# jaco267/polar-code-pytorch-sionna

Hardware: NVIDIA B200
Metric: decoded_info_throughput_sc_n1024 (higher is better)
Workload: dtype f32

## Files before the change

### polar-code-pytorch-sionna_b200/csrc/polar_sc5.cu

```cuda
#include <atomic>
#include <mutex>

#include "polar_common.cuh"
#include "polar_internal.h"

namespace polar {

#if !defined(POLAR_F_BOXPLUS)
namespace {
__global__ void nsmid_kernel(unsigned *out) {
  unsigned v;
  asm volatile("mov.u32 %0, %%nsmid;" : "=r"(v));
  *out = v;
}
std::mutex g_scr_mu;
std::atomic<float *> g_scr_buf[64];
}

int sc_scratch_init(int device) {
  if (device < 0 || device >= 64) return set_error(POLAR_EINVAL, "init: bad device %d", device);
  std::lock_guard<std::mutex> lk(g_scr_mu);
  if (g_scr_buf[device].load(std::memory_order_acquire)) return POLAR_OK;
  unsigned *d_n = nullptr, h_n = 0;
  POLAR_CUDA(cudaMalloc(&d_n, sizeof(unsigned)));
  nsmid_kernel<<<1, 1>>>(d_n);
  const cudaError_t e = cudaMemcpy(&h_n, d_n, sizeof(unsigned), cudaMemcpyDeviceToHost);
  cudaFree(d_n);
  if (e != cudaSuccess) return set_error(POLAR_ECUDA, "init: %s", cudaGetErrorString(e));
  if (h_n == 0 || h_n > 1024) return set_error(POLAR_ECUDA, "init: implausible %%nsmid = %u", h_n);
  void *p = nullptr;
  if (cudaMalloc(&p, (size_t)h_n * kScScratchPerSm) != cudaSuccess) {
    (void)cudaGetLastError();
    return set_error(POLAR_ENOMEM, "init: cudaMalloc of the %zu-byte SC stage scratch failed", (size_t)h_n * kScScratchPerSm);
  }
  g_scr_buf[device].store((float *)p, std::memory_order_release);
  return POLAR_OK;
}
float *sc_scratch() {
  int dev = 0;
  if (cudaGetDevice(&dev) != cudaSuccess || dev < 0 || dev >= 64) return nullptr;
  return g_scr_buf[dev].load(std::memory_order_acquire);
}
#endif

__device__ unsigned long long g_sc5_dbg[8];

namespace {

constexpr unsigned FULLMASK = 0xFFFFFFFFu;
constexpr int kSlotFloats = 1024, kSlotBytes = 4096;
constexpr int kSlots = 6;
constexpr int kHeaderBytes = 1024;

#define SC5_T(slot)                                                                   \
  do {                                                                                \
    if (DBG && threadIdx.x == 0 && blockIdx.x == 0) {                                 \
      const long long t__ = clock64(); g_sc5_dbg[slot] += (unsigned long long)(t__ - tlast); tlast = t__; \
    }                                                                                 \
  } while (0)

struct Ctl {
  unsigned long long bar[8 * kSlots];
  uint32_t tm_addr;
  uint32_t pad[3];
};
static_assert(sizeof(Ctl) + 128 + 8 <= kHeaderBytes, "sc5: header");

struct Sc5Layout {
  int nw, nws, n64, stride, slots;
  size_t fmask_off, nz_off, warp_off, per_warp, beta_off, total;
};
__host__ __device__ inline Sc5Layout sc5_layout(int m, int warps, int slots) {
  Sc5Layout l;
  const int n = 1 << m;
  l.nw = n >> 5; l.nws = l.nw + 1; l.n64 = n >> 7; l.slots = slots;
  l.stride = 128 + 4;
  l.fmask_off = (sizeof(Ctl) + 15) / 16 * 16;
  l.nz_off = l.fmask_off + (size_t)l.nw * 4;
  l.warp_off = (l.nz_off + (size_t)l.n64 + 1023) / 1024 * 1024;
  l.beta_off = (size_t)slots * kSlotBytes > (size_t)32 * l.stride * 4 ? (size_t)slots * kSlotBytes : (size_t)32 * l.stride * 4;
  l.per_warp = (l.beta_off + (size_t)32 * l.nws * 4 + 127) / 128 * 128;
  l.total = l.warp_off + (size_t)warps * l.per_warp;
  return l;
}

PDEV uint32_t smem_u32(const void *p) { return (uint32_t)__cvta_generic_to_shared(p); }
PDEV void mbar_init(unsigned long long *bar, uint32_t count) {
  asm volatile("mbarrier.init.shared::cta.b64 [%0], %1;" ::"r"(smem_u32(bar)), "r"(count) : "memory");
}
PDEV void mbar_expect_tx(unsigned long long *bar, uint32_t bytes) {
  asm volatile("mbarrier.arrive.expect_tx.shared::cta.b64 _, [%0], %1;" ::"r"(smem_u32(bar)), "r"(bytes) : "memory");
}
PDEV void mbar_wait(unsigned long long *bar, uint32_t parity) {
  asm volatile(
      "{\n\t"
      ".reg .pred P1;\n\t"
      "SC5_WAIT:\n\t"
      "mbarrier.try_wait.parity.shared::cta.b64 P1, [%0], %1, %2;\n\t"
      "@P1 bra SC5_DONE;\n\t"
      "bra SC5_WAIT;\n\t"
      "SC5_DONE:\n\t"
      "}" ::"r"(smem_u32(bar)), "r"(parity), "r"(0x989680u) : "memory");
}
PDEV void bulk_g2s(void *dst, const void *src, uint32_t bytes, unsigned long long *bar, uint64_t policy) {
  asm volatile("cp.async.bulk.shared::cluster.global.mbarrier::complete_tx::bytes.L2::cache_hint [%0], [%1], %2, [%3], %4;"
               ::"r"(smem_u32(dst)), "l"(src), "r"(bytes), "r"(smem_u32(bar)), "l"(policy) : "memory");
}
PDEV uint64_t l2_policy_evict_last() {
  uint64_t p; asm volatile("createpolicy.fractional.L2::evict_last.b64 %0, 1.0;" : "=l"(p)); return p;
}
PDEV uint64_t l2_policy_evict_first() {
  uint64_t p; asm volatile("createpolicy.fractional.L2::evict_first.b64 %0, 1.0;" : "=l"(p)); return p;
}
PDEV uint64_t l2_policy_evict_normal() {
  uint64_t p; asm volatile("createpolicy.fractional.L2::evict_normal.b64 %0, 1.0;" : "=l"(p)); return p;
}
PDEV void stg4_hint(float *p, const float4 v, uint64_t policy) {
  asm volatile("st.global.L2::cache_hint.v4.f32 [%0], {%1, %2, %3, %4}, %5;"
               ::"l"(p), "f"(v.x), "f"(v.y), "f"(v.z), "f"(v.w), "l"(policy) : "memory");
}
PDEV float4 lds4(const float *p) { return *reinterpret_cast<const float4 *>(p); }
PDEV void sts4(float *p, float4 v) { *reinterpret_cast<float4 *>(p) = v; }
PDEV float4 f4(const float4 a, const float4 b) {
  float4 o;
  o.x = f_minsum(a.x, b.x); o.y = f_minsum(a.y, b.y); o.z = f_minsum(a.z, b.z); o.w = f_minsum(a.w, b.w);
  return o;
}
PDEV float4 f4nc(const float4 a, const float4 b) {
  float4 o;
  o.x = f_minsum_noclip(a.x, b.x); o.y = f_minsum_noclip(a.y, b.y); o.z = f_minsum_noclip(a.z, b.z); o.w = f_minsum_noclip(a.w, b.w);
  return o;
}
PDEV float4 f4neg(const float4 a, const float4 b) {
  float4 o;
  o.x = f_minsum_neg(a.x, b.x); o.y = f_minsum_neg(a.y, b.y); o.z = f_minsum_neg(a.z, b.z); o.w = f_minsum_neg(a.w, b.w);
  return o;
}
PDEV float4 g4(const float4 a, const float4 b, const uint32_t bits) {
  float4 o;
  o.x = g_minsum(a.x, b.x, (bits << 31) & 0x80000000u);
  o.y = g_minsum(a.y, b.y, (bits << 30) & 0x80000000u);
  o.z = g_minsum(a.z, b.z, (bits << 29) & 0x80000000u);
  o.w = g_minsum(a.w, b.w, (bits << 28) & 0x80000000u);
  return o;
}
PDEV float gneg(float a, float b, uint32_t signmask) { return u2f(f2u(a) ^ signmask ^ 0x80000000u) - b; }
PDEV float4 g4neg(const float4 a, const float4 b, const uint32_t bits) {
  float4 o;
  o.x = gneg(a.x, b.x, (bits << 31) & 0x80000000u);
  o.y = gneg(a.y, b.y, (bits << 30) & 0x80000000u);
  o.z = gneg(a.z, b.z, (bits << 29) & 0x80000000u);
  o.w = gneg(a.w, b.w, (bits << 28) & 0x80000000u);
  return o;
}

PDEV void tmem_st8(uint32_t taddr, const float4 a, const float4 b) {
  asm volatile("tcgen05.st.sync.aligned.32x32b.x8.b32 [%0], {%1, %2, %3, %4, %5, %6, %7, %8};"
               ::"r"(taddr), "r"(f2u(a.x)), "r"(f2u(a.y)), "r"(f2u(a.z)), "r"(f2u(a.w)), "r"(f2u(b.x)), "r"(f2u(b.y)),
               "r"(f2u(b.z)), "r"(f2u(b.w)) : "memory");
}
PDEV void tmem_st4(uint32_t taddr, const float4 a) {
  asm volatile("tcgen05.st.sync.aligned.32x32b.x4.b32 [%0], {%1, %2, %3, %4};"
               ::"r"(taddr), "r"(f2u(a.x)), "r"(f2u(a.y)), "r"(f2u(a.z)), "r"(f2u(a.w)) : "memory");
}
PDEV void tmem_wait_st() { asm volatile("tcgen05.wait::st.sync.aligned;" ::: "memory"); }
struct Tm8 { uint32_t r[8]; };
PDEV void tmem_ld8_issue(uint32_t taddr, Tm8 &v) {
  asm volatile("tcgen05.ld.sync.aligned.32x32b.x8.b32 {%0, %1, %2, %3, %4, %5, %6, %7}, [%8];"
               : "=r"(v.r[0]), "=r"(v.r[1]), "=r"(v.r[2]), "=r"(v.r[3]), "=r"(v.r[4]), "=r"(v.r[5]), "=r"(v.r[6]), "=r"(v.r[7])
               : "r"(taddr) : "memory");
}
PDEV void tmem_ld_wait(Tm8 &a, Tm8 &b) {
  asm volatile("tcgen05.wait::ld.sync.aligned;"
               : "+r"(a.r[0]), "+r"(a.r[1]), "+r"(a.r[2]), "+r"(a.r[3]), "+r"(a.r[4]), "+r"(a.r[5]), "+r"(a.r[6]), "+r"(a.r[7]),
                 "+r"(b.r[0]), "+r"(b.r[1]), "+r"(b.r[2]), "+r"(b.r[3]), "+r"(b.r[4]), "+r"(b.r[5]), "+r"(b.r[6]), "+r"(b.r[7])
               :: "memory");
}
PDEV float4 tm_lo(const Tm8 &v) { return make_float4(u2f(v.r[0]), u2f(v.r[1]), u2f(v.r[2]), u2f(v.r[3])); }
PDEV float4 tm_hi(const Tm8 &v) { return make_float4(u2f(v.r[4]), u2f(v.r[5]), u2f(v.r[6]), u2f(v.r[7])); }

template <int D, bool FIRST_G, bool FROM_CH, int NS>
__device__ __noinline__ void descent(const float *__restrict__ src, const int nvalid, const uint32_t *beta, const int nws,
                                     const int left_word, float *scr, const uint32_t tm_base, float *Lw, const uint32_t bar_a,
                                     uint32_t &par, const int lane, const bool discard) {
  constexpr int NB = 1 << D;
  constexpr int HB = NB / 2;
  constexpr int SRC = 256 * NB;
  constexpr bool WIDE = D <= 2;
  constexpr int CPS = D == 1 ? 2 : 1;
  constexpr int NQ = WIDE ? 1 : (1 << (D - 3));
  constexpr int K = WIDE ? 32 / CPS : 64 * NQ;
  constexpr int T1 = 8 + D - 1;
  const uint64_t pol_src = FROM_CH ? l2_policy_evict_first() : (D == 1 ? l2_policy_evict_last() : l2_policy_evict_normal());
  const uint64_t pol_s9 = l2_policy_evict_last(), pol_sx = l2_policy_evict_normal();
  if (!FROM_CH) asm volatile("fence.proxy.async.global;" ::: "memory");
  asm volatile("fence.proxy.async.shared::cta;" ::: "memory");
  __syncwarp();
  const uint32_t slot_a = smem_u32(Lw);

  auto issue2 = [&](const int k, const int ring) {
    if (WIDE) {
      if (lane < 2) {
        const int s = ring + lane;
        int c = (k + lane) * CPS;
        if (FROM_CH && c >= nvalid) c = nvalid - 1;
        asm volatile("mbarrier.arrive.expect_tx.shared::cta.b64 _, [%0], %1;" ::"r"(bar_a + 8 * s), "r"(4096) : "memory");
        asm volatile("cp.async.bulk.shared::cluster.global.mbarrier::complete_tx::bytes.L2::cache_hint [%0], [%1], %2, [%3], %4;"
                     ::"r"(slot_a + 4096 * s), "l"(src + (size_t)c * SRC), "r"(4096), "r"(bar_a + 8 * s), "l"(pol_src) : "memory");
      }
    } else {
      if (lane < 2)
        asm volatile("mbarrier.arrive.expect_tx.shared::cta.b64 _, [%0], %1;" ::"r"(bar_a + 8 * (ring + lane)), "r"(4096) : "memory");
      __syncwarp();
      if (lane < 16) {
        const int h = lane >> 3, p = lane & 7, s = ring + h;
        int c = k / (2 * NQ);
        const int q = (k >> 1) % NQ;
        if (FROM_CH && c >= nvalid) c = nvalid - 1;
        const int blk = (p & 3) + 4 * q + ((p >> 2) ? HB : 0);
        asm volatile("cp.async.bulk.shared::cluster.global.mbarrier::complete_tx::bytes.L2::cache_hint [%0], [%1], %2, [%3], %4;"
                     ::"r"(slot_a + 4096 * s + 512 * p), "l"(src + (size_t)c * SRC + blk * 256 + h * 128), "r"(512), "r"(bar_a + 8 * s),
                     "l"(pol_src) : "memory");
      }
    }
  };
  auto wait = [&](const int s) -> const float * {
    asm volatile(
        "{\n\t"
        ".reg .pred P1;\n\t"
        "SC5_WAIT:\n\t"
        "mbarrier.try_wait.parity.shared::cta.b64 P1, [%0], %1, %2;\n\t"
        "@P1 bra SC5_DONE;\n\t"
        "bra SC5_WAIT;\n\t"
        "SC5_DONE:\n\t"
        "}" ::"r"(bar_a + 8 * s), "r"((par >> s) & 1u), "r"(0x989680u) : "memory");
    return Lw + s * kSlotFloats;
  };

#pragma unroll
  for (int r = 0; r < NS; r += 2) issue2(r, r);
  int ring = 0;
  const int col = 4 * lane;
  float *st1 = scr + (size_t)32 * ((1 << T1) - 512) + col;
  const uint32_t *bp = beta + left_word + (col >> 5);
  const int sh = col & 31;
  const float *dp = src + lane * 32;
  if constexpr (WIDE) {
    constexpr int CW = 2 * CPS;
    int tcol = 0;
#pragma unroll 1
    for (int k = 0; k < K; k += 2) {
      const float *sl[2];
      sl[0] = wait(ring); sl[1] = wait(ring + 1);
      float4 v[CW][2][NB];
#pragma unroll
      for (int u = 0; u < CW; ++u)
#pragma unroll
        for (int e = 0; e < 2; ++e)
#pragma unroll
          for (int i = 0; i < NB; ++i) v[u][e][i] = lds4(sl[u / CPS] + (u % CPS) * SRC + i * 256 + col + 128 * e);
      float4 out[CW][2];
#pragma unroll
      for (int u = 0; u < CW; ++u) {
#pragma unroll
        for (int e = 0; e < 2; ++e) {
          float4 r1[HB];
#pragma unroll
          for (int i = 0; i < HB; ++i) {
            if (FIRST_G) {
              const uint32_t bits = bp[u * nws + i * 8 + e * 4] >> sh;
              r1[i] = FROM_CH ? g4neg(v[u][e][i], v[u][e][i + HB], bits) : g4(v[u][e][i], v[u][e][i + HB], bits);
            } else {
              r1[i] = FROM_CH ? f4neg(v[u][e][i], v[u][e][i + HB]) : f4(v[u][e][i], v[u][e][i + HB]);
            }
            if (D >= 2) stg4_hint(st1 + u * (1 << T1) + i * 256 + e * 128, r1[i], T1 == 9 ? pol_s9 : pol_sx);
          }
          if (D == 2) out[u][e] = FIRST_G ? f4(r1[0], r1[HB - 1]) : f4nc(r1[0], r1[HB - 1]);
          else out[u][e] = r1[0];
        }
      }
      if (!FROM_CH && discard) {
        asm volatile("discard.global.L2 [%0], 128;" ::"l"(dp) : "memory");
        asm volatile("discard.global.L2 [%0], 128;" ::"l"(dp + 1024) : "memory");
      }
      st1 += CW << T1; bp += CW * nws; dp += 2048;
      __syncwarp();
      par ^= 3u << ring;
      if (k + NS < K) issue2(k + NS, ring);
#pragma unroll
      for (int u = 0; u < CW; ++u) tmem_st8(tm_base + tcol + 8 * u, out[u][0], out[u][1]);
      tcol += 8 * CW;
      ring = (ring + 2 == NS) ? 0 : ring + 2;
    }
  } else {
    const int piece = (lane >> 2) & 7, line = lane & 3;
    dp = src + ((piece & 3) + ((piece >> 2) ? HB : 0)) * 256 + line * 32;
#pragma unroll 1
    for (int c = 0; c < 32; ++c) {
      float4 R[2][HB];
#pragma unroll
      for (int q = 0; q < NQ; ++q) {
        const int k = (c * NQ + q) * 2;
        const float *sl[2];
        sl[0] = wait(ring); sl[1] = wait(ring + 1);
        float4 v[2][8];
#pragma unroll
        for (int h = 0; h < 2; ++h)
#pragma unroll
          for (int p = 0; p < 8; ++p) v[h][p] = lds4(sl[h] + p * 128 + col);
#pragma unroll
        for (int h = 0; h < 2; ++h) {
#pragma unroll
          for (int t = 0; t < 4; ++t) {
            const int blk = 4 * q + t;
            if (FIRST_G) {
              const uint32_t bits = bp[blk * 8 + h * 4] >> sh;
              R[h][blk] = FROM_CH ? g4neg(v[h][t], v[h][4 + t], bits) : g4(v[h][t], v[h][4 + t], bits);
            } else {
              R[h][blk] = FROM_CH ? f4neg(v[h][t], v[h][4 + t]) : f4(v[h][t], v[h][4 + t]);
            }
            stg4_hint(st1 + blk * 256 + h * 128, R[h][blk], T1 == 9 ? pol_s9 : pol_sx);
          }
        }
        if (!FROM_CH && discard) {
          asm volatile("discard.global.L2 [%0], 128;" ::"l"(dp + 4 * q * 256) : "memory");
          asm volatile("discard.global.L2 [%0], 128;" ::"l"(dp + 4 * q * 256 + 128) : "memory");
        }
        __syncwarp();
        par ^= 3u << ring;
        if (k + NS < K) issue2(k + NS, ring);
        ring = (ring + 2 == NS) ? 0 : ring + 2;
      }
#pragma unroll
      for (int lv = D - 1; lv >= 1; --lv) {
        const int half = 1 << (lv - 1);
        float *stl = scr + (size_t)32 * ((1 << (8 + lv - 1)) - 512) + (size_t)c * (1 << (8 + lv - 1)) + col;
#pragma unroll
        for (int h = 0; h < 2; ++h)
#pragma unroll
          for (int i = 0; i < half; ++i) {
            R[h][i] = (FIRST_G && lv == D - 1) ? f4(R[h][i], R[h][i + half]) : f4nc(R[h][i], R[h][i + half]);
            if (lv - 1 >= 1) stg4_hint(stl + i * 256 + h * 128, R[h][i], (8 + lv - 1) == 9 ? pol_s9 : pol_sx);
          }
      }
      tmem_st8(tm_base + 8 * c, R[0][0], R[1][0]);
      st1 += 1 << T1; bp += nws; dp += SRC;
    }
  }
  tmem_wait_st();
  __syncwarp();
}

template <bool IS_G>
PDEV void step_tmem(float *L, const uint32_t *beta, const int stride, const int nws, const int lane, const uint32_t tm_base,
                    const int left_word) {
  const int j = lane << 2;
  const uint32_t *bp = beta + left_word + (j >> 5);
  const int sh = j & 31;
  float *dst = L + j;
  Tm8 a0, a1, a2, a3, b0, b1, b2, b3;
  auto issue4 = [&](const int k0, Tm8 &v0, Tm8 &v1, Tm8 &v2, Tm8 &v3) {
    tmem_ld8_issue(tm_base + 8 * k0, v0);
    tmem_ld8_issue(tm_base + 8 * (k0 + 1), v1);
    tmem_ld8_issue(tm_base + 8 * (k0 + 2), v2);
    tmem_ld8_issue(tm_base + 8 * (k0 + 3), v3);
  };
  auto compute4 = [&](const int k0, const Tm8 &v0, const Tm8 &v1, const Tm8 &v2, const Tm8 &v3) {
#pragma unroll
    for (int r = 0; r < 4; ++r) {
      const Tm8 &v = r == 0 ? v0 : r == 1 ? v1 : r == 2 ? v2 : v3;
      const float4 a = tm_lo(v), b = tm_hi(v);
      float4 o;
      if (IS_G) o = g4(a, b, bp[(k0 + r) * nws] >> sh);
      else o = f4(a, b);
      sts4(dst + (k0 + r) * stride, o);
    }
  };
  issue4(0, a0, a1, a2, a3);
#pragma unroll 1
  for (int k0 = 0; k0 < 32; k0 += 8) {
    tmem_ld_wait(a0, a1); tmem_ld_wait(a2, a3);
    issue4(k0 + 4, b0, b1, b2, b3);
    compute4(k0, a0, a1, a2, a3);
    tmem_ld_wait(b0, b1); tmem_ld_wait(b2, b3);
    if (k0 + 8 < 32) issue4(k0 + 8, a0, a1, a2, a3);
    compute4(k0 + 4, b0, b1, b2, b3);
  }
}

PDEV uint64_t tree64(const float (&x)[64], uint64_t fm) {
  uint32_t bl = 0, bc = 0;
#pragma unroll 1
  for (int h = 0; h < 2; ++h) {
    const uint32_t fmc = h ? (uint32_t)(fm >> 32) : (uint32_t)fm;
    if (fmc == FULLMASK) { bc = 0; continue; }
    float y[32];
#pragma unroll
    for (int j = 0; j < 32; ++j)
      y[j] = h ? g_minsum(x[j], x[j + 32], (bl << (31 - j)) & 0x80000000u) : f_minsum(x[j], x[j + 32]);
    bc = BetaTree<5>::run(y, fmc);
    if (h == 0) bl = bc;
  }
  return (uint64_t)(bl ^ bc) | ((uint64_t)bc << 32);
}
PDEV uint4 bottom128(const float *node, uint64_t fm0, uint64_t fm1) {
  uint64_t bl = 0, bc = 0;
#pragma unroll 1
  for (int h = 0; h < 2; ++h) {
    const uint64_t fmc = h ? fm1 : fm0;
    if (fmc == ~0ull) { bc = 0; continue; }
    float x[64];
#pragma unroll
    for (int q = 0; q < 16; ++q) {
      const float4 a = lds4(node + 4 * q), b = lds4(node + 64 + 4 * q);
      const float4 o = h ? g4(a, b, (uint32_t)(bl >> (4 * q))) : f4(a, b);
      x[4 * q] = o.x; x[4 * q + 1] = o.y; x[4 * q + 2] = o.z; x[4 * q + 3] = o.w;
    }
    bc = tree64(x, fmc);
    if (h == 0) bl = bc;
  }
  const uint64_t lo = bl ^ bc;
  return make_uint4((uint32_t)lo, (uint32_t)(lo >> 32), (uint32_t)bc, (uint32_t)(bc >> 32));
}

template <int M, int NS, bool DBG>
__global__ void __launch_bounds__(256, 1) sc5_kernel(const float *__restrict__ logit, const uint32_t *__restrict__ fmask_g,
                                                     int64_t B, int64_t nbatches, float *scratch, size_t scratch_per_sm,
                                                     int scr_discard, uint32_t *__restrict__ u_packed, float *__restrict__ u_info,
                                                     const int32_t *__restrict__ info_pos, int k) {
  static_assert(M >= 10 && M <= 13, "sc5: n = 1024 .. 8192");
  extern __shared__ __align__(128) unsigned char smem_raw[];
  constexpr int N = 1 << M, NW = N >> 5, NWS = NW + 1, N64 = N >> 7, stride = 132;
  const int tid = threadIdx.x, lane = tid & 31, warp = __shfl_sync(FULLMASK, tid >> 5, 0), nwarps = blockDim.x >> 5;
  Sc5Layout lay = sc5_layout(M, nwarps, NS);
  Ctl *P = reinterpret_cast<Ctl *>(smem_raw);
  uint32_t *fmask = reinterpret_cast<uint32_t *>(smem_raw + lay.fmask_off);
  unsigned char *nz = smem_raw + lay.nz_off;
  float *L = reinterpret_cast<float *>(smem_raw + lay.warp_off + (size_t)warp * lay.per_warp);
  uint32_t *beta = reinterpret_cast<uint32_t *>(reinterpret_cast<unsigned char *>(L) + lay.beta_off);
  const uint32_t bar_a = smem_u32(&P->bar[kSlots * warp]);
  uint32_t par = 0;

  if (warp == 0) {
    asm volatile("tcgen05.alloc.cta_group::1.sync.aligned.shared::cta.b32 [%0], %1;"
                 ::"r"(smem_u32(&P->tm_addr)), "n"(512) : "memory");
    asm volatile("tcgen05.relinquish_alloc_permit.cta_group::1.sync.aligned;" ::: "memory");
  }
  if (tid == 0) {
    for (int s = 0; s < 8 * kSlots; ++s) mbar_init(&P->bar[s], 1);
    asm volatile("fence.mbarrier_init.release.cluster;" ::: "memory");
    asm volatile("fence.proxy.async.shared::cta;" ::: "memory");
  }
  asm volatile("tcgen05.fence::before_thread_sync;" ::: "memory");
  for (int i = tid; i < NW; i += blockDim.x) fmask[i] = __ldg(fmask_g + i);
  __syncthreads();
  asm volatile("tcgen05.fence::after_thread_sync;" ::: "memory");
  const uint32_t tm_base = P->tm_addr + ((uint32_t)((warp & 3) * 32) << 16) + (uint32_t)((warp >> 2) * 256);
  for (int i = tid; i < N64; i += blockDim.x)
    nz[i] = (fmask[4 * i] & fmask[4 * i + 1] & fmask[4 * i + 2] & fmask[4 * i + 3]) == FULLMASK;
  __syncthreads();

  uint32_t smid;
  asm volatile("mov.u32 %0, %%smid;" : "=r"(smid));
  float *scr = scratch + (size_t)smid * (scratch_per_sm / 4) + (size_t)warp * 32 * (N - 512);
  long long tlast = DBG ? clock64() : 0;
  const long long tstart = tlast;
  const int64_t wstride = (int64_t)gridDim.x * nwarps;
  for (int64_t batch = (int64_t)warp * gridDim.x + blockIdx.x; batch < nbatches; batch += wstride) {
    const int64_t cw0 = batch * 32;
    const int nvalid = (int)((B - cw0) < 32 ? (B - cw0) : 32);
#pragma unroll 1
    for (int i = 0; i < N64; ++i) {
      const bool zero_blk = __shfl_sync(FULLMASK, (int)nz[i], 0) != 0;
      if ((i & 1) == 0) {
        const int S = (i == 0) ? M : 7 + (__ffs(i) - 1);
        const bool dead = __shfl_sync(FULLMASK, (int)(nz[i] & nz[i + 1]), 0) != 0;
        if (S == M) {
          descent<M - 8, false, true, NS>(logit + cw0 * (int64_t)N, nvalid, beta, NWS, 0, scr, tm_base, L, bar_a, par, lane, false);
        } else if (S == M - 1) {
          descent<M - 8, true, true, NS>(logit + cw0 * (int64_t)N, nvalid, beta, NWS, 0, scr, tm_base, L, bar_a, par, lane, false);
        } else {
          const int left_word = 4 * (i - (1 << (S - 7)));
          const float *sp = scr + (size_t)32 * ((1 << (S + 1)) - 512);
          const bool dis = scr_discard != 0;
          switch (S) {
            case 8: if (!dead) descent<1, true, false, NS>(sp, 32, beta, NWS, left_word, scr, tm_base, L, bar_a, par, lane, dis); break;
            case 9: if (M > 10) descent<(M > 10 ? 2 : 1), true, false, NS>(sp, 32, beta, NWS, left_word, scr, tm_base, L, bar_a, par, lane, dis); break;
            case 10: if (M > 11) descent<(M > 11 ? 3 : 1), true, false, NS>(sp, 32, beta, NWS, left_word, scr, tm_base, L, bar_a, par, lane, dis); break;
            case 11: if (M > 12) descent<(M > 12 ? 4 : 1), true, false, NS>(sp, 32, beta, NWS, left_word, scr, tm_base, L, bar_a, par, lane, dis); break;
            default: break;
          }
        }
        __syncwarp();
        if (S >= M - 1) SC5_T(0); else SC5_T(1);
        if (!zero_blk) {
          step_tmem<false>(L, beta, stride, NWS, lane, tm_base, 0);
          __syncwarp();
        }
        SC5_T(2);
      } else if (!zero_blk) {
        step_tmem<true>(L, beta, stride, NWS, lane, tm_base, 4 * (i - 1));
        __syncwarp();
        SC5_T(2);
      }
      if (zero_blk) {
        for (int q = lane; q < 128; q += 32) beta[(q >> 2) * NWS + 4 * i + (q & 3)] = 0u;
      } else {
        const uint32_t *fmw = fmask + 4 * i;
        const uint32_t f0 = __shfl_sync(FULLMASK, fmw[0], 0), f1 = __shfl_sync(FULLMASK, fmw[1], 0);
        const uint32_t f2 = __shfl_sync(FULLMASK, fmw[2], 0), f3 = __shfl_sync(FULLMASK, fmw[3], 0);
        const uint4 b = bottom128(L + lane * stride, (uint64_t)f0 | ((uint64_t)f1 << 32), (uint64_t)f2 | ((uint64_t)f3 << 32));
        uint32_t *bp = beta + lane * NWS + 4 * i;
        bp[0] = b.x; bp[1] = b.y; bp[2] = b.z; bp[3] = b.w;
      }
      __syncwarp();
      SC5_T(3);
      {
        uint32_t *bw = beta + lane * NWS;
        int lv = 0, a = i;
        while (lv < M - 7 && ((a >> lv) & 1)) {
          const int nwd = 4 << lv, left = a - (1 << lv);
#pragma unroll 1
          for (int w = 0; w < nwd; w += 4) {
            const uint32_t r0 = bw[4 * a + w], r1 = bw[4 * a + w + 1], r2 = bw[4 * a + w + 2], r3 = bw[4 * a + w + 3];
            const uint32_t l0 = bw[4 * left + w], l1 = bw[4 * left + w + 1], l2 = bw[4 * left + w + 2], l3 = bw[4 * left + w + 3];
            bw[4 * left + w] = l0 ^ r0; bw[4 * left + w + 1] = l1 ^ r1; bw[4 * left + w + 2] = l2 ^ r2; bw[4 * left + w + 3] = l3 ^ r3;
          }
          a = left; ++lv;
        }
        __syncwarp();
      }
      SC5_T(4);
    }
    if constexpr (NW <= 64) {
      uint32_t *bw = beta + lane * NWS;
      uint32_t w[NW];
#pragma unroll
      for (int t = 0; t < NW; ++t) w[t] = ptransform<5>(bw[t]);
#pragma unroll
      for (int st = 0; st < M - 5; ++st)
#pragma unroll
        for (int t = 0; t < NW; ++t)
          if (!(t & (1 << st))) w[t] ^= w[t + (1 << st)];
      if (u_packed && lane < nvalid) {
        uint32_t *dst = u_packed + (cw0 + lane) * NW;
        if ((reinterpret_cast<uintptr_t>(dst) & 15) == 0) {
#pragma unroll
          for (int t = 0; t < NW; t += 4) __stcs(reinterpret_cast<uint4 *>(dst + t), make_uint4(w[t], w[t + 1], w[t + 2], w[t + 3]));
        } else {
#pragma unroll
          for (int t = 0; t < NW; ++t) dst[t] = w[t];
        }
      }
      if (u_info) {
#pragma unroll
        for (int t = 0; t < NW; ++t) bw[t] = w[t];
      }
      __syncwarp();
    } else {
      for (int q = lane; q < 32 * NW; q += 32) {
        const int c = q / NW, w = q % NW;
        beta[c * NWS + w] = ptransform<5>(beta[c * NWS + w]);
      }
      __syncwarp();
#pragma unroll 1
      for (int st = 0; st < M - 5; ++st) {
        for (int q = lane; q < 32 * (NW / 2); q += 32) {
          const int c = q / (NW / 2), r = q % (NW / 2);
          const int w = ((r >> st) << (st + 1)) | (r & ((1 << st) - 1));
          beta[c * NWS + w] ^= beta[c * NWS + w + (1 << st)];
        }
        __syncwarp();
      }
      if (u_packed) {
        for (int q = lane; q < 32 * NW; q += 32) {
          const int c = q / NW, w = q % NW;
          if (c < nvalid) u_packed[(cw0 + c) * NW + w] = beta[c * NWS + w];
        }
      }
    }
    if (u_info) {
      if ((k & 3) == 0 && (reinterpret_cast<uintptr_t>(u_info) & 15) == 0 && (reinterpret_cast<uintptr_t>(info_pos) & 15) == 0) {
        const int k4 = k >> 2;
        const int4 *ip = reinterpret_cast<const int4 *>(info_pos);
        for (int c = 0; c < nvalid; ++c) {
          float4 *row = reinterpret_cast<float4 *>(u_info + (cw0 + c) * (int64_t)k);
          const uint32_t *bw = beta + c * NWS;
          for (int t4 = lane; t4 < k4; t4 += 32) {
            const int4 p = __ldg(ip + t4);
            float4 o;
            o.x = u2f((0u - ((bw[p.x >> 5] >> (p.x & 31)) & 1u)) & 0x3f800000u);
            o.y = u2f((0u - ((bw[p.y >> 5] >> (p.y & 31)) & 1u)) & 0x3f800000u);
            o.z = u2f((0u - ((bw[p.z >> 5] >> (p.z & 31)) & 1u)) & 0x3f800000u);
            o.w = u2f((0u - ((bw[p.w >> 5] >> (p.w & 31)) & 1u)) & 0x3f800000u);
            __stcs(row + t4, o);
          }
        }
      } else {
        for (int q = lane; q < nvalid * k; q += 32) {
          const int c = q / k, t = q - c * k;
          const int p = __ldg(info_pos + t);
          u_info[(cw0 + c) * (int64_t)k + t] = (float)((beta[c * NWS + (p >> 5)] >> (p & 31)) & 1u);
        }
      }
    }
    __syncwarp();
    SC5_T(5);
    if (DBG && tid == 0 && blockIdx.x == 0) g_sc5_dbg[7] += 1;
  }
  if (DBG && tid == 0 && blockIdx.x == 0) g_sc5_dbg[6] += (unsigned long long)(clock64() - tstart);
  asm volatile("tcgen05.fence::before_thread_sync;" ::: "memory");
  __syncthreads();
  if (warp == 0)
    asm volatile("tcgen05.dealloc.cta_group::1.sync.aligned.b32 %0, %1;" ::"r"(P->tm_addr), "n"(512) : "memory");
}

template <int M>
int launch_sc5_t(const float *logit, const uint32_t *fmask, int64_t B, uint32_t *u_packed, float *u_info,
                 const int32_t *info_pos, int k, int warps, cudaStream_t st) {
  const int max_smem = device_max_smem_optin();
  constexpr int N = 1 << M;
  int wmax = 8;
  if (warps <= 0 || warps > wmax) warps = wmax;
  while (warps > 1 && (sc5_layout(M, warps, 4).total > (size_t)max_smem ||
                       (size_t)warps * 32 * (N - 512) * 4 > kScScratchPerSm)) --warps;
  int ns = env_int("POLAR_SC5_SLOTS", 6);
  if (ns != 6 || sc5_layout(M, warps, 6).total > (size_t)max_smem) ns = 4;
  const Sc5Layout lay = sc5_layout(M, warps, ns);
  if (lay.total > (size_t)max_smem) return set_error(POLAR_ENOMEM, "sc: n=%d needs more shared memory per CTA than the device has", N);
  float *scratch = sc_scratch();
  if (!scratch)
    return set_error(POLAR_EINVAL, "sc: n=%d needs the per-device stage scratch -- call polar_init(device) once before decoding", N);
  const bool dbg = env_int("POLAR_SC3_DBG", 0) != 0;
  auto kern = dbg ? (ns == 6 ? sc5_kernel<M, 6, true> : sc5_kernel<M, 4, true>) : (ns == 6 ? sc5_kernel<M, 6, false> : sc5_kernel<M, 4, false>);
  size_t smem = lay.total;
  if (smem < (size_t)116 * 1024) smem = (size_t)116 * 1024;
  POLAR_CUDA(cudaFuncSetAttribute(kern, cudaFuncAttributeMaxDynamicSharedMemorySize, (int)smem));
  const int sms = device_sm_count();
  const int64_t nbatches = (B + 31) / 32;
  int64_t grid = (nbatches + warps - 1) / warps;
  if (grid > sms) grid = sms;
  if (grid < 1) grid = 1;
  kern<<<(unsigned)grid, warps * 32, smem, st>>>(logit, fmask, B, nbatches, scratch,
                                              (size_t)warps * 32 * (N - 512) * 4,
                                                      env_int("POLAR_SC4_DISCARD", 1), u_packed, u_info, info_pos, k);
  count_launch();
  POLAR_CHECK_LAUNCH("sc5_kernel");
  return POLAR_OK;
}

}

int launch_sc5(const float *logit, const uint32_t *fmask, int n, int64_t B, uint32_t *u_packed, float *u_info,
               const int32_t *info_pos, int k, int warps, cudaStream_t st) {
  switch (ilog2(n)) {
    case 10: return launch_sc5_t<10>(logit, fmask, B, u_packed, u_info, info_pos, k, warps, st);
    case 11: return launch_sc5_t<11>(logit, fmask, B, u_packed, u_info, info_pos, k, warps, st);
    case 12: return launch_sc5_t<12>(logit, fmask, B, u_packed, u_info, info_pos, k, warps, st);
    case 13: return launch_sc5_t<13>(logit, fmask, B, u_packed, u_info, info_pos, k, warps, st);
    default: return set_error(POLAR_EINVAL, "sc5: n=%d not supported by this mapping", n);
  }
}

}

extern "C" int polar_sc5_debug_read(unsigned long long *h_out8) {
  unsigned long long z[8] = {0, 0, 0, 0, 0, 0, 0, 0};
  if (cudaMemcpyFromSymbol(h_out8, polar::g_sc5_dbg, sizeof(z)) != cudaSuccess) return POLAR_ECUDA;
  if (cudaMemcpyToSymbol(polar::g_sc5_dbg, z, sizeof(z)) != cudaSuccess) return POLAR_ECUDA;
  return POLAR_OK;
}
```

Measured before the change: 248.4.

## Decode 8-leaf special nodes (Rep, SPC, Rate-1, Rep-SPC) with closed-form rules

Adds a per-8-leaf node type table, built once in shared memory from the frozen mask. Types are Rate-0, Rep, SPC, Rate-1 and Rep-SPC. The bottom SC tree now uses a NodeTree recursion that decodes these nodes directly instead of walking the full binary BetaTree down to single leaves. This cuts the serial f/g recursion and per-bit decisions in the bottom 128-leaf stage. In exchange it adds extra shared-memory layout, shuffles of the type words, and fallback paths (warp-wide votes) when the Rate-1 shortcut does not apply.

```diff
diff --git a/polar-code-pytorch-sionna_b200/csrc/polar_sc5.cu b/polar-code-pytorch-sionna_b200/csrc/polar_sc5.cu
--- a/polar-code-pytorch-sionna_b200/csrc/polar_sc5.cu
+++ b/polar-code-pytorch-sionna_b200/csrc/polar_sc5.cu
@@ -3,6 +3,7 @@
 
 #include "polar_common.cuh"
 #include "polar_internal.h"
+#include "polar_sc_nodes.cuh"
 
 namespace polar {
 
@@ -68,7 +69,7 @@
 
 struct Sc5Layout {
   int nw, nws, n64, stride, slots;
-  size_t fmask_off, nz_off, warp_off, per_warp, beta_off, total;
+  size_t fmask_off, nz_off, nt_off, warp_off, per_warp, beta_off, total;
 };
 __host__ __device__ inline Sc5Layout sc5_layout(int m, int warps, int slots) {
   Sc5Layout l;
@@ -77,7 +78,8 @@
   l.stride = 128 + 4;
   l.fmask_off = (sizeof(Ctl) + 15) / 16 * 16;
   l.nz_off = l.fmask_off + (size_t)l.nw * 4;
-  l.warp_off = (l.nz_off + (size_t)l.n64 + 1023) / 1024 * 1024;
+  l.nt_off = (l.nz_off + (size_t)l.n64 + 15) / 16 * 16;
+  l.warp_off = (l.nt_off + (size_t)(n >> 3) + 1023) / 1024 * 1024;
   l.beta_off = (size_t)slots * kSlotBytes > (size_t)32 * l.stride * 4 ? (size_t)slots * kSlotBytes : (size_t)32 * l.stride * 4;
   l.per_warp = (l.beta_off + (size_t)32 * l.nws * 4 + 127) / 128 * 128;
   l.total = l.warp_off + (size_t)warps * l.per_warp;
@@ -388,22 +390,23 @@
   }
 }
 
-PDEV uint64_t tree64(const float (&x)[64], uint64_t fm) {
+PDEV uint64_t tree64(const float (&x)[64], uint64_t fm, uint64_t ty) {
   uint32_t bl = 0, bc = 0;
 #pragma unroll 1
   for (int h = 0; h < 2; ++h) {
     const uint32_t fmc = h ? (uint32_t)(fm >> 32) : (uint32_t)fm;
+    const uint32_t tyc = h ? (uint32_t)(ty >> 32) : (uint32_t)ty;
     if (fmc == FULLMASK) { bc = 0; continue; }
     float y[32];
 #pragma unroll
     for (int j = 0; j < 32; ++j)
       y[j] = h ? g_minsum(x[j], x[j + 32], (bl << (31 - j)) & 0x80000000u) : f_minsum(x[j], x[j + 32]);
-    bc = BetaTree<5>::run(y, fmc);
+    bc = NodeTree<5>::run(y, fmc, tyc);
     if (h == 0) bl = bc;
   }
   return (uint64_t)(bl ^ bc) | ((uint64_t)bc << 32);
 }
-PDEV uint4 bottom128(const float *node, uint64_t fm0, uint64_t fm1) {
+PDEV uint4 bottom128(const float *node, uint64_t fm0, uint64_t fm1, uint64_t ty0, uint64_t ty1) {
   uint64_t bl = 0, bc = 0;
 #pragma unroll 1
   for (int h = 0; h < 2; ++h) {
@@ -416,7 +419,7 @@
       const float4 o = h ? g4(a, b, (uint32_t)(bl >> (4 * q))) : f4(a, b);
       x[4 * q] = o.x; x[4 * q + 1] = o.y; x[4 * q + 2] = o.z; x[4 * q + 3] = o.w;
     }
-    bc = tree64(x, fmc);
+    bc = tree64(x, fmc, h ? ty1 : ty0);
     if (h == 0) bl = bc;
   }
   const uint64_t lo = bl ^ bc;
@@ -436,6 +439,8 @@
   Ctl *P = reinterpret_cast<Ctl *>(smem_raw);
   uint32_t *fmask = reinterpret_cast<uint32_t *>(smem_raw + lay.fmask_off);
   unsigned char *nz = smem_raw + lay.nz_off;
+  unsigned char *nt = smem_raw + lay.nt_off;
+  const uint32_t *ntw = reinterpret_cast<const uint32_t *>(nt);
   float *L = reinterpret_cast<float *>(smem_raw + lay.warp_off + (size_t)warp * lay.per_warp);
   uint32_t *beta = reinterpret_cast<uint32_t *>(reinterpret_cast<unsigned char *>(L) + lay.beta_off);
   const uint32_t bar_a = smem_u32(&P->bar[kSlots * warp]);
@@ -458,6 +463,8 @@
   const uint32_t tm_base = P->tm_addr + ((uint32_t)((warp & 3) * 32) << 16) + (uint32_t)((warp >> 2) * 256);
   for (int i = tid; i < N64; i += blockDim.x)
     nz[i] = (fmask[4 * i] & fmask[4 * i + 1] & fmask[4 * i + 2] & fmask[4 * i + 3]) == FULLMASK;
+#pragma unroll 1
+  for (int i = tid; i < N / 8; i += blockDim.x) nt[i] = (unsigned char)node8_type(fmask[i >> 2] >> (8 * (i & 3)));
   __syncthreads();
 
   uint32_t smid;
@@ -509,7 +516,11 @@
         const uint32_t *fmw = fmask + 4 * i;
         const uint32_t f0 = __shfl_sync(FULLMASK, fmw[0], 0), f1 = __shfl_sync(FULLMASK, fmw[1], 0);
         const uint32_t f2 = __shfl_sync(FULLMASK, fmw[2], 0), f3 = __shfl_sync(FULLMASK, fmw[3], 0);
-        const uint4 b = bottom128(L + lane * stride, (uint64_t)f0 | ((uint64_t)f1 << 32), (uint64_t)f2 | ((uint64_t)f3 << 32));
+        const uint32_t *ntb = ntw + 4 * i;
+        const uint32_t t0 = __shfl_sync(FULLMASK, ntb[0], 0), t1 = __shfl_sync(FULLMASK, ntb[1], 0);
+        const uint32_t t2 = __shfl_sync(FULLMASK, ntb[2], 0), t3 = __shfl_sync(FULLMASK, ntb[3], 0);
+        const uint4 b = bottom128(L + lane * stride, (uint64_t)f0 | ((uint64_t)f1 << 32), (uint64_t)f2 | ((uint64_t)f3 << 32),
+                                  (uint64_t)t0 | ((uint64_t)t1 << 32), (uint64_t)t2 | ((uint64_t)t3 << 32));
         uint32_t *bp = beta + lane * NWS + 4 * i;
         bp[0] = b.x; bp[1] = b.y; bp[2] = b.z; bp[3] = b.w;
       }
diff --git a/polar-code-pytorch-sionna_b200/csrc/polar_sc_nodes.cuh b/polar-code-pytorch-sionna_b200/csrc/polar_sc_nodes.cuh
--- /dev/null
+++ b/polar-code-pytorch-sionna_b200/csrc/polar_sc_nodes.cuh
@@ -0,0 +1,152 @@
+#pragma once
+#include "polar_common.cuh"
+
+namespace polar {
+
+enum : uint32_t {
+  kN8Generic = 0,
+  kN8Rate0 = 1,
+  kN8Rep = 2,
+  kN8Spc = 3,
+  kN8Rate1 = 4,
+  kN8RepSpc = 5,
+};
+PHD uint32_t node8_type(uint32_t fm8) {
+  const uint32_t m = fm8 & 0xFFu;
+  return m == 0xFFu ? kN8Rate0 : m == 0x7Fu ? kN8Rep : m == 0x01u ? kN8Spc : m == 0x00u ? kN8Rate1 : m == 0x17u ? kN8RepSpc
+                                                                                                                : kN8Generic;
+}
+
+PDEV bool rep4_u(const float (&x)[4]) { return ((x[0] + x[2]) + (x[1] + x[3])) <= 0.0f; }
+
+template <bool CL>
+PDEV uint32_t spc4_beta(const float (&x)[4]) {
+  const float a0 = CL ? f_minsum_noclip(x[0], x[2]) : f_minsum(x[0], x[2]);
+  const float a1 = CL ? f_minsum_noclip(x[1], x[3]) : f_minsum(x[1], x[3]);
+  const float s0 = x[0] + x[2], d0 = x[2] - x[0], s1 = x[1] + x[3], d1 = x[3] - x[1];
+  const bool u1 = (a0 + a1) <= 0.0f;
+  const float b0 = u1 ? d0 : s0, b1 = u1 ? d1 : s1;
+  const float l2 = f_minsum_noclip(b0, b1);
+  const float sb = b0 + b1, db = b1 - b0;
+  const bool u2 = l2 <= 0.0f;
+  const float l3 = u2 ? db : sb;
+  const bool u3 = l3 <= 0.0f;
+  const bool p2 = u2 != u3;
+  return (uint32_t)(u1 != p2) | ((uint32_t)(u1 != u3) << 1) | ((uint32_t)p2 << 2) | ((uint32_t)u3 << 3);
+}
+
+template <bool CL>
+PDEV uint32_t node8_beta(const float (&x)[8], uint32_t fm, uint32_t ty) {
+  switch (ty) {
+    case kN8Rep: {
+      float y[4];
+#pragma unroll
+      for (int j = 0; j < 4; ++j) y[j] = x[j] + x[j + 4];
+      return rep4_u(y) ? 0xFFu : 0u;
+    }
+    case kN8Rate1: {
+      uint32_t b;
+      const bool ok = rate1_beta<3>(x, b);
+      if (__all_sync(0xFFFFFFFFu, ok)) return b;
+      break;
+    }
+    case kN8Spc: {
+      float y[4], sd[4], df[4];
+#pragma unroll
+      for (int j = 0; j < 4; ++j) {
+        y[j] = CL ? f_minsum_noclip(x[j], x[j + 4]) : f_minsum(x[j], x[j + 4]);
+        sd[j] = x[j] + x[j + 4]; df[j] = x[j + 4] - x[j];
+      }
+      const uint32_t bl = spc4_beta<true>(y);
+#pragma unroll
+      for (int j = 0; j < 4; ++j) y[j] = ((bl >> j) & 1u) ? df[j] : sd[j];
+      uint32_t br;
+      const bool ok = rate1_beta<2>(y, br);
+      if (__all_sync(0xFFFFFFFFu, ok)) return (bl ^ br) | (br << 4);
+      break;
+    }
+    case kN8RepSpc: {
+      float y[4], sd[4], df[4];
+#pragma unroll
+      for (int j = 0; j < 4; ++j) {
+        y[j] = CL ? f_minsum_noclip(x[j], x[j + 4]) : f_minsum(x[j], x[j + 4]);
+        sd[j] = x[j] + x[j + 4]; df[j] = x[j + 4] - x[j];
+      }
+      const bool ul = rep4_u(y);
+#pragma unroll
+      for (int j = 0; j < 4; ++j) y[j] = ul ? df[j] : sd[j];
+      const uint32_t br = spc4_beta<false>(y);
+      return ((ul ? 0xFu : 0u) ^ br) | (br << 4);
+    }
+    default: break;
+  }
+  return BetaTree<3, CL>::run(x, fm);
+}
+
+template <int T, bool CL = false>
+struct NodeTree;
+template <bool CL>
+struct NodeTree<3, CL> {
+  PDEV static uint32_t run(const float (&x)[8], uint32_t fm, uint32_t ty) { return node8_beta<CL>(x, fm & 0xFFu, ty & 0xFFu); }
+};
+template <bool CL>
+struct NodeTree<4, CL> {
+  PDEV static uint32_t run(const float (&x)[16], uint32_t fm, uint32_t ty) {
+    fm &= 0xFFFFu;
+    if (fm == 0xFFFFu) return 0;
+    if (fm == 0) {
+      uint32_t b;
+      const bool ok = rate1_beta<4>(x, b);
+      if (__all_sync(0xFFFFFFFFu, ok)) return b;
+    }
+    float y[8];
+    uint32_t bl = 0, br = 0;
+    if ((fm & 0xFFu) != 0xFFu) {
+#pragma unroll
+      for (int j = 0; j < 8; ++j) y[j] = CL ? f_minsum_noclip(x[j], x[j + 8]) : f_minsum(x[j], x[j + 8]);
+      bl = NodeTree<3, true>::run(y, fm, ty);
+    }
+    if ((fm >> 8) != 0xFFu) {
+#pragma unroll
+      for (int j = 0; j < 8; ++j) y[j] = g_minsum(x[j], x[j + 8], (bl << (31 - j)) & 0x80000000u);
+      br = NodeTree<3, false>::run(y, fm >> 8, ty >> 8);
+    }
+    return (bl ^ br) | (br << 8);
+  }
+};
+template <int T, bool CL>
+struct NodeTree {
+  static constexpr int N = 1 << T, H = N / 2;
+  static constexpr uint32_t FULL = (N == 32) ? 0xFFFFFFFFu : ((1u << N) - 1u);
+  static constexpr uint32_t HALF = (1u << H) - 1u;
+  static_assert(T == 5, "NodeTree: the type word holds 4 nodes of 8 leaves");
+  PDEV static uint32_t run(const float (&x)[N], uint32_t fm, uint32_t ty) {
+    fm &= FULL;
+    if (fm == FULL) return 0;
+    if (fm == 0) {
+      uint32_t b;
+      const bool ok = rate1_beta<T>(x, b);
+      if (__all_sync(0xFFFFFFFFu, ok)) return b;
+    }
+    float y[H];
+    uint32_t bl = 0, bc = 0;
+#pragma unroll 1
+    for (int h = 0; h < 2; ++h) {
+      const uint32_t fmc = (h == 0) ? (fm & HALF) : (fm >> H);
+      const uint32_t tyc = (h == 0) ? ty : (ty >> H);
+      if (fmc == HALF) { bc = 0; continue; }
+      if (h == 0) {
+#pragma unroll
+        for (int j = 0; j < H; ++j) y[j] = CL ? f_minsum_noclip(x[j], x[j + H]) : f_minsum(x[j], x[j + H]);
+      } else {
+#pragma unroll
+        for (int j = 0; j < H; ++j) y[j] = g_minsum(x[j], x[j + H], (bl << (31 - j)) & 0x80000000u);
+      }
+      bc = NodeTree<T - 1>::run(y, fmc, tyc);
+      if (h == 0) bl = bc;
+    }
+    return (bl ^ bc) | (bc << H);
+  }
+};
+
+}
```

New measurement: 239.2, median of 6. 0.963x the previous value.
